# facebookresearch/video-long-term-feature-banks

Hardware: AMD Instinct MI355X
Metric: clips/sec fwd+bwd R50-I3D-NL+LFB-NL, 32x224^2 synthetic (higher is better)
Workload: dtype mix; 1 GPU; ava_r50_lfb_nl fwd+bwd+allreduce+sgd, 8 clips/GPU (global batch 8), RoIs/clip ~ U{1..5} (33 on rank 0), 32x224x224 clips; parallelism=dp1

## Files before the change

video-long-term-feature-banks_amd/csrc/vlfb_gemm.hip:

```cpp
#include "vlfb_conv_plan.h"
#include "vlfb_gemm_nt.h"

namespace vlfb {
namespace {

__device__ __forceinline__ uint32_t word_of(const uint4& v, int i) {
  return i == 0 ? v.x : i == 1 ? v.y : i == 2 ? v.z : v.w;
}
__device__ __forceinline__ void transpose_block(const uint4 (&in)[8], uint4 (&out)[8], bf16_t) {
#pragma unroll
  for (int c = 0; c < 8; ++c) {
    uint32_t o[4];
#pragma unroll
    for (int q = 0; q < 4; ++q) {
      const uint32_t w0 = word_of(in[2 * q], c >> 1), w1 = word_of(in[2 * q + 1], c >> 1);
      o[q] = (c & 1) ? ((w0 >> 16) | (w1 & 0xffff0000u)) : ((w0 & 0xffffu) | (w1 << 16));
    }
    out[c] = make_uint4(o[0], o[1], o[2], o[3]);
  }
}
__device__ __forceinline__ void transpose_block(const uint4 (&in)[8], uint4 (&out)[8], f16_t) {
  transpose_block(in, out, bf16_t());
}
__device__ __forceinline__ void transpose_block(const uint4 (&in)[4], uint4 (&out)[4], float) {
// ... 561 lines not shown
  float* slab = p.ws + (long long)split * ((long long)p.Ncols * p.ldo);
#pragma unroll
  for (int j = 0; j < kStemCT; ++j) {
    const int ct = ct0 + j;
    if (ct >= ncts) continue;
#pragma unroll
    for (int i = 0; i < 4; ++i) {
      const int co = i * 16 + l15;
      *reinterpret_cast<float4*>(slab + (long long)co * p.ldo + ct * 16 + g * 4) =
          make_float4(acc[j][i][0], acc[j][i][1], acc[j][i][2], acc[j][i][3]);
    }
  }
}

template <typename OutT, int G, int CL>
__global__ __launch_bounds__(CL * G) void wgrad_reduce_kernel(const float* ws, char* O, const float* rowscale,
                                                              long long n, int ldo, int splits, float alpha,
                                                              int accumulate, const float* __restrict__ ws_b = nullptr,
                                                              float* __restrict__ dbias = nullptr, int nb = 0, int wblocks = 0) {
  if (ws_b != nullptr && (int)blockIdx.x >= wblocks) {
    const int i = ((int)blockIdx.x - wblocks) * (CL * G) + (int)threadIdx.x;
    if (i < nb) {
      float s = 0.f;
      for (int k = 0; k < splits; ++k) s += ws_b[(long long)k * nb + i];
      dbias[i] = s * alpha * (rowscale ? rowscale[i] : 1.f);
    }
    return;
  }
  __shared__ float4 part[G > 1 ? (G - 1) * CL : 1];
  const int lane = threadIdx.x % CL, g = threadIdx.x / CL;
  const long long i = ((long long)blockIdx.x * CL + lane) * 4;
  float4 s = {0.f, 0.f, 0.f, 0.f};
  if (i < n) {
    const float* src = ws + i;
    int k = g;
    for (; k + 3 * G < splits; k += 4 * G) {
      float4 t0 = *reinterpret_cast<const float4*>(src + (long long)k * n);
      float4 t1 = *reinterpret_cast<const float4*>(src + (long long)(k + G) * n);
      float4 t2 = *reinterpret_cast<const float4*>(src + (long long)(k + 2 * G) * n);
      float4 t3 = *reinterpret_cast<const float4*>(src + (long long)(k + 3 * G) * n);
      s.x += (t0.x + t1.x) + (t2.x + t3.x); s.y += (t0.y + t1.y) + (t2.y + t3.y);
      s.z += (t0.z + t1.z) + (t2.z + t3.z); s.w += (t0.w + t1.w) + (t2.w + t3.w);
    }
    for (; k < splits; k += G) {
      float4 t = *reinterpret_cast<const float4*>(src + (long long)k * n);
      s.x += t.x; s.y += t.y; s.z += t.z; s.w += t.w;
    }
  }
  if (G > 1) {
    if (g > 0) part[(g - 1) * CL + lane] = s;
    __syncthreads();
    if (g == 0) {
#pragma unroll
      for (int j = 0; j < G - 1; ++j) {
        float4 t = part[j * CL + lane];
        s.x += t.x; s.y += t.y; s.z += t.z; s.w += t.w;
      }
    }
  }
  if (g == 0 && i < n) {
    float rs = alpha * (rowscale ? rowscale[i / ldo] : 1.f);
    float v[4] = {s.x * rs, s.y * rs, s.z * rs, s.w * rs};
    if (accumulate) {
#pragma unroll
      for (int r = 0; r < 4; ++r) v[r] += ld_elem<OutT>(O, i + r);
    }
    store4<OutT>(O, i, v, 4, true);
  }
}

__global__ void wgrad_bias_reduce_kernel(const float* __restrict__ ws_b, float* __restrict__ out,
                                         const float* __restrict__ rowscale, int n, int splits, float alpha) {
  const int i = blockIdx.x * blockDim.x + threadIdx.x;
  if (i >= n) return;
  float s = 0.f;
  for (int k = 0; k < splits; ++k) s += ws_b[(long long)k * n + i];
  out[i] = s * alpha * (rowscale ? rowscale[i] : 1.f);
}

template <auto Kernel>
int launch_k(const Plan& pl, hipStream_t s, const char* what) {
  return launch_lds<Kernel, 80 * 1024>(pl.grid, dim3(pl.threads), pl.lds, s, what, pl.gp);
}
template <typename T, typename OutT, int BM, int BN, bool IDENT, bool DGRAD, bool PACKW, int RB, bool PRE, int NW>
int launch_nt_shape(const Plan& pl, hipStream_t s, const char* what) {
  if constexpr (!IDENT && !PACKW) {
    if constexpr (DGRAD && sizeof(T) == 2) {
      if (pl.w2i) return launch_k<gemm_nt_kernel<T, OutT, BM, BN, IDENT, DGRAD, PACKW, RB, PRE, NW, 2, true, false, true>>(pl, s, what);
    }
    if (pl.ut) return launch_k<gemm_nt_kernel<T, OutT, BM, BN, IDENT, DGRAD, PACKW, RB, PRE, NW, 2, true>>(pl, s, what);
  }
  return launch_k<gemm_nt_kernel<T, OutT, BM, BN, IDENT, DGRAD, PACKW, RB, PRE, NW, 2, false>>(pl, s, what);
}

template <typename T, typename OutT, bool IDENT, bool DGRAD, bool PACKW>
int launch_nt(const Plan& pl, hipStream_t s, const char* what) {
  constexpr bool BF = sizeof(T) == 2;
  constexpr bool CAN_PRE = BF && sizeof(OutT) == 2 && !PACKW;
  constexpr int NW = BF ? 8 : 4;
  if (pl.bn == 64) {
    if (CAN_PRE && pl.pre) return launch_nt_shape<T, OutT, 128, 64, IDENT, DGRAD, PACKW, 128, CAN_PRE, NW>(pl, s, what);
    return launch_nt_shape<T, OutT, 128, 64, IDENT, DGRAD, PACKW, 128, false, NW>(pl, s, what);
  }
  if (CAN_PRE && pl.pre) return launch_nt_shape<T, OutT, 128, 128, IDENT, DGRAD, PACKW, 128, CAN_PRE, NW>(pl, s, what);
  return launch_nt_shape<T, OutT, 128, 128, IDENT, DGRAD, PACKW, 128, false, NW>(pl, s, what);
}
template <typename T, typename OutT, bool IDENT, bool PACKW>
int launch_tn(const Plan& pl, hipStream_t s, const char* what) {
  if (pl.bm == 128 && pl.bn == 128) return launch_k<gemm_tn_kernel<T, OutT, 128, 128, IDENT, PACKW>>(pl, s, what);
  if (pl.bm == 64 && pl.bn == 256) return launch_k<gemm_tn_kernel<T, OutT, 64, 256, IDENT, PACKW>>(pl, s, what);
  if (pl.bm == 64 && pl.bn == 128) return launch_k<gemm_tn_kernel<T, OutT, 64, 128, IDENT, PACKW>>(pl, s, what);
  if (pl.bm == 128 && pl.bn == 64) return launch_k<gemm_tn_kernel<T, OutT, 128, 64, IDENT, PACKW>>(pl, s, what);
  return launch_k<gemm_tn_kernel<T, OutT, 64, 64, IDENT, PACKW>>(pl, s, what);
}

template <typename T, typename OutT, bool IDENT, bool PACKW, bool SP>
int launch_tn_tr_as(const Plan& pl, hipStream_t s, const char* what) {
  if (pl.bm == 128 && pl.bn == 128) return launch_k<gemm_tn_tr_kernel<T, OutT, 128, 128, IDENT, PACKW, 8, SP>>(pl, s, what);
  if (pl.bm == 64 && pl.bn == 128) return launch_k<gemm_tn_tr_kernel<T, OutT, 64, 128, IDENT, PACKW, 4, SP>>(pl, s, what);
  if (pl.bm == 128 && pl.bn == 64) return launch_k<gemm_tn_tr_kernel<T, OutT, 128, 64, IDENT, PACKW, 4, SP>>(pl, s, what);
  return launch_k<gemm_tn_tr_kernel<T, OutT, 64, 64, IDENT, PACKW, 4, SP>>(pl, s, what);
}
template <typename T, typename OutT, bool SP = false>
int launch_tn_tr(const Plan& pl, hipStream_t s, const char* what) {
  return pl.ident ? launch_tn_tr_as<T, OutT, true, false, SP>(pl, s, what)
         : pl.packw ? launch_tn_tr_as<T, OutT, false, true, SP>(pl, s, what)
                    : launch_tn_tr_as<T, OutT, false, false, SP>(pl, s, what);
}

template <typename T>
int launch_stem_wgrad(const Plan& pl, hipStream_t s) {
  return launch_lds<stem_wgrad_kernel<T>, 160 * 1024>(pl.grid, dim3(512), pl.lds, s, "conv wgrad (stem) kernel", pl.gp);
}

template <typename T, typename OutT>
int launch_tiled(const vlfb_conv_desc* d, const Plan& pl, hipStream_t s) {
  if constexpr (sizeof(T) == 2) {
    if (pl.family == Family::tn_tr) return launch_tn_tr<T, OutT>(pl, s, "conv wgrad (tr) kernel");
  }
  const char* what = "conv kernel";
  if (d->mode == VLFB_CONV_WGRAD) {
    if (pl.ident) return launch_tn<T, OutT, true, false>(pl, s, what);
    if (pl.packw) return launch_tn<T, OutT, false, true>(pl, s, what);
    return launch_tn<T, OutT, false, false>(pl, s, what);
  }
  if (d->mode == VLFB_CONV_DGRAD) {
    if (pl.ident) return launch_nt<T, OutT, true, false, false>(pl, s, what);
    return launch_nt<T, OutT, false, true, false>(pl, s, what);
  }
  if (pl.ident) return launch_nt<T, OutT, true, false, false>(pl, s, what);
  if (pl.packw) return launch_nt<T, OutT, false, false, true>(pl, s, what);
  return launch_nt<T, OutT, false, false, false>(pl, s, what);
}

int launch_plan(const vlfb_conv_desc* d, const Plan& pl, hipStream_t s) {
  const GP& g = pl.gp;
  const bool out_f32 = d->out_dtype == VLFB_F32;
  switch (pl.family) {
    case Family::tn:
    case Family::tn_tr:
    case Family::nt:
      if (d->dtype == VLFB_F32) return launch_tiled<float, float>(d, pl, s);
      if (d->dtype == VLFB_F16) return out_f32 ? launch_tiled<f16_t, float>(d, pl, s) : launch_tiled<f16_t, f16_t>(d, pl, s);
      return out_f32 ? launch_tiled<bf16_t, float>(d, pl, s) : launch_tiled<bf16_t, bf16_t>(d, pl, s);
    case Family::tn8: return launch_tn8(g, pl.grid, d->dtype, out_f32, s);
    case Family::stem_wgrad: VLFB_WITH_T16(d->dtype, return launch_stem_wgrad<T16>(pl, s));
    case Family::wgrad_rows: return launch_wgrad_rows(g, pl.splits, pl.lds, d->dtype, s);
    case Family::wgrad_rows_fat: return launch_wgrad_rows_fat(g, pl.splits, d->dtype, s);
    case Family::tn_split: return launch_tn_split(g, pl.bm, pl.bn, pl.ident, pl.packw, pl.grid, pl.lds, s);
    case Family::tn_tr_planes: return launch_tn_tr<bf16_t, float, true>(pl, s, "conv wgrad (planes) kernel");
    case Family::nt8:
      return launch_nt8(g, pl.bm, pl.bn, pl.nt8_mode, d->dtype, out_f32, (unsigned)(d->batch > 0 ? d->batch : 1), s);
    case Family::nt_stream: return launch_nts(g, pl.nts_mode, d->dtype, s);
    case Family::conv_rows64: return launch_conv_rows64(g, d->mode, d->dtype, s);
    case Family::stem_fprop: return launch_stem_fprop(g, d->dtype, s);
    case Family::nt_skinny: return launch_skinny_nt(g, d->dtype, out_f32, s);
    case Family::nt_skinny_split: return launch_skinny_nt_split(g, s);
    case Family::nt_split: return launch_nt_split(g, pl.sp, pl.bn, pl.sp_kind, pl.ut != 0, pl.grid, pl.lds, s);
    case Family::nt_planes: return launch_nt_planes(g, pl.sp, pl.bn, pl.sp_kind, pl.grid, pl.lds, s);
    case Family::nt_pair: return launch_nt_pair(g, pl.bn, pl.ident, pl.pre != 0, out_f32, pl.grid, pl.lds, s);
    case Family::nt8_pair: return launch_nt8_pair(g, pl.bm, pl.bn, pl.nt8_mode, out_f32, s);
    case Family::stem_fprop_pair: return launch_stem_fprop_pair(g, s);
  }
  return set_error(VLFB_ERR_ARG, "conv: plan without a kernel family");
}

}
// ... 39 lines not shown
      const int64_t* v = static_cast<const int64_t*>(arg);
      const int64_t n = vlfb_class_ap_voc_workspace_bytes_impl(v[0], v[1]);
      if (n < 0) set_error(VLFB_ERR_ARG, "query_workspace: class_ap_voc needs 1 <= n <= %d and cols >= 1", VLFB_CLASS_AP_MAX_N);
      return n;
    }
    default: set_error(VLFB_ERR_ARG, "query_workspace: unknown op %d", op); return -1;
  }
}

extern "C" int vlfb_conv_run(const vlfb_conv_desc* d, const void* A, const void* B, const void* P,
                             void* O, const float* bias, const float* rowscale, const void* R,
                             const void* Mask, void* workspace, int64_t workspace_bytes,
                             vlfb_stream_t stream) {
  return vlfb_conv_run_planes(d, A, B, P, O, bias, rowscale, R, Mask, workspace, workspace_bytes, nullptr, stream);
}

static int conv_run_impl(const vlfb_conv_desc* d, const void* A, const void* B, const void* P,
                         void* O, const float* bias, const float* rowscale, const void* R,
                         const void* Mask, void* workspace, int64_t workspace_bytes, void* O_planes, float* dbias,
                         vlfb_stream_t stream, const void* R_lo = nullptr, void* O_lo = nullptr);

extern "C" int vlfb_conv_run_args(const vlfb_conv_desc* d, const vlfb_conv_args* a, vlfb_stream_t stream) {
  VLFB_REQUIRE(d && a, "conv_run_args: descriptor and arguments are required");
  VLFB_REQUIRE(!d->wgrad_bias == !a->dbias, "conv_run_args: dbias goes with desc.wgrad_bias");
  return conv_run_impl(d, a->A, a->B, a->P, a->O, a->bias, a->rowscale, a->R, a->Mask, a->workspace, a->workspace_bytes,
                       a->O_planes, a->dbias, stream, a->R_lo, a->O_lo);
}

extern "C" int vlfb_conv_run_planes(const vlfb_conv_desc* d, const void* A, const void* B, const void* P,
                                    void* O, const float* bias, const float* rowscale, const void* R,
                                    const void* Mask, void* workspace, int64_t workspace_bytes, void* O_planes,
                                    vlfb_stream_t stream) {
  VLFB_REQUIRE(!d->wgrad_bias, "conv: a descriptor with wgrad_bias runs through vlfb_conv_run_wgrad_bias");
  return conv_run_impl(d, A, B, P, O, bias, rowscale, R, Mask, workspace, workspace_bytes, O_planes, nullptr, stream);
}

extern "C" int vlfb_conv_run_wgrad_bias(const vlfb_conv_desc* d, const void* A, const void* P, void* O, float* dbias,
                                        const float* rowscale, void* workspace, int64_t workspace_bytes,
                                        vlfb_stream_t stream) {
  VLFB_REQUIRE(d->mode == VLFB_CONV_WGRAD && d->wgrad_bias && dbias, "conv_run_wgrad_bias: a WGRAD descriptor with wgrad_bias = 1 and dbias");
  return conv_run_impl(d, A, nullptr, P, O, nullptr, rowscale, nullptr, nullptr, workspace, workspace_bytes, nullptr, dbias, stream);
}

static int conv_run_impl(const vlfb_conv_desc* d, const void* A, const void* B, const void* P,
                         void* O, const float* bias, const float* rowscale, const void* R,
                         const void* Mask, void* workspace, int64_t workspace_bytes, void* O_planes, float* dbias,
                         vlfb_stream_t stream, const void* R_lo, void* O_lo) {
  Plan pl;
  int rc = cached_plan(d, &pl);
  if (rc != VLFB_OK) return rc;
  const bool h2 = d->math == VLFB_MATH_F16X3;
  const bool sp_pair = pl.sp && d->out_dtype == VLFB_F16;
  VLFB_REQUIRE(!sp_pair || (O_lo && (!R || R_lo)), "conv: a two-plane fp16 output needs O_lo (and R_lo with R)");
  VLFB_REQUIRE(!h2 || d->out_dtype == VLFB_F32 || O_lo, "conv: F16X3 math with a 16-bit output writes two planes (O, O_lo)");
  VLFB_REQUIRE(!h2 || !Mask, "conv: F16X3 launches take no mask");
  const bool copy16 = O_lo && !R_lo && !pl.sp && !h2 && is16(d->dtype) && d->out_dtype == VLFB_F32 && d->mode != VLFB_CONV_WGRAD;
  if ((R_lo || O_lo) && !sp_pair && !(h2 && d->out_dtype == VLFB_F32 && !R_lo)) {
    VLFB_REQUIRE(d->mode != VLFB_CONV_WGRAD && is16(d->dtype) && (d->out_dtype == d->dtype || copy16) && !pl.sp,
                 "conv: R_lo / O_lo belong to 16-bit FPROP / DGRAD launches with 16-bit outputs (O_lo alone: also with an fp32 output)");
    VLFB_REQUIRE(!R_lo || R, "conv: R_lo without R");
    VLFB_REQUIRE(pl.gp.vec_epi, "conv: R_lo / O_lo need 16-byte aligned output rows");
  }
  VLFB_REQUIRE(A && O, "conv: A and O are required");
  if (d->mode == VLFB_CONV_WGRAD) VLFB_REQUIRE(P != nullptr, "conv: WGRAD needs P");
  else VLFB_REQUIRE(B != nullptr, "conv: FPROP/DGRAD need B");
  VLFB_REQUIRE(d->bias_mode == VLFB_BIAS_NONE || bias != nullptr, "conv: bias_mode set but bias is NULL");
  if (pl.ws_elems > 0 && (workspace == nullptr || workspace_bytes < pl.ws_elems * 4))
    return set_error(VLFB_ERR_WORKSPACE, "conv: split WGRAD needs %lld workspace bytes, got %lld",
                     (long long)pl.ws_elems * 4, (long long)workspace_bytes);
  VLFB_REQUIRE((d->o_planes > 0) == (O_planes != nullptr), "conv: O_planes goes with desc.o_planes");
  rc = resolve_for_operands(d, &pl, R != nullptr, Mask != nullptr, R_lo != nullptr, O_lo != nullptr);
  if (rc != VLFB_OK) return rc;
  GP& g = pl.gp;
  g.A = (const char*)A; g.B = (const char*)B; g.P = (const char*)P; g.O = (char*)O;
  g.bias = bias; g.rowscale = rowscale; g.R = (const char*)R; g.Mask = (const char*)Mask;
  g.ws = (float*)workspace;
  g.OP = (char*)O_planes;
  g.dbias = pl.bias_fused ? dbias : nullptr;
  g.R2 = (const char*)R_lo; g.O2 = (char*)O_lo;
  g.pair_io = sp_pair ? 1 : 0;
  static const int nt_epi = env_int("VLFB_NT_EPI", 1);
  const bool wide_epi = h2 || pl.sp || pl.w2i || d->dt == 0 || d->out_dtype == VLFB_F32 || R_lo || O_lo;
  g.nt_epi = nt_epi >= 2 || (nt_epi == 1 && wide_epi);
  hipStream_t s = (hipStream_t)stream;
  rc = launch_plan(d, pl, s);
  if (rc != VLFB_OK) return rc;
  if (dbias && !pl.bias_fused) {
    VLFB_REQUIRE(!d->a_planes, "conv: wgrad_bias with pre-split operands is not supported (pass the fp32 operands)");
    const int slabs = colsum_slabs(d->dtype, g.M, d->Cn);
    float* part = g.ws + (pl.splits > 1 ? (long long)pl.splits * ((long long)d->Cn * g.ldo) : 0);
    rc = colsum_partials(P, d->dtype, g.M, d->Cn, g.ldp, part, s);
    if (rc != VLFB_OK) return rc;
    hipLaunchKernelGGL(wgrad_bias_reduce_kernel, dim3((unsigned)((d->Cn + 63) / 64)), dim3(64), 0, s, part, dbias, rowscale,
                       d->Cn, slabs, d->alpha);
  }
  const float* bias_rows = (dbias && pl.bias_fused && pl.splits > 1) ? g.ws + (long long)pl.splits * ((long long)d->Cn * g.ldo) : nullptr;
  if (pl.splits > 1) {
    const long long n = (long long)d->Cn * g.K;
    VLFB_REQUIRE(n % 4 == 0, "conv: split WGRAD output size must be a multiple of 4");
    const int G = pl.splits >= 32 ? 16 : pl.splits >= 8 ? 4 : 1;
#define VLFB_REDUCE(OT, GG, CC)                                                                                         \
  do {                                                                                                                  \
    const unsigned wblocks = (unsigned)((n / 4 + CC - 1) / CC);                                                         \
    const unsigned bblocks = bias_rows ? (unsigned)((d->Cn + CC * GG - 1) / (CC * GG)) : 0u;                            \
    hipLaunchKernelGGL((wgrad_reduce_kernel<OT, GG, CC>), dim3(wblocks + bblocks), dim3(CC * GG), 0, s, g.ws, g.O,     \
                       rowscale, n, g.ldo, pl.splits, d->alpha, d->accumulate, bias_rows, bias_rows ? dbias : nullptr,  \
                       (int)d->Cn, (int)wblocks);                                                                       \
  } while (0)
    with_elem(d->out_dtype, [&](auto t) {
      using OT = decltype(t);
      if (G == 16) VLFB_REDUCE(OT, 16, 16); else if (G == 4) VLFB_REDUCE(OT, 4, 64); else VLFB_REDUCE(OT, 1, 64);
    });
#undef VLFB_REDUCE
    return check_launch("wgrad reduce");
  }
  return VLFB_OK;
}
```

video-long-term-feature-banks_amd/csrc/vlfb_gemm_common.h:

```cpp
#pragma once
#include "vlfb_common.h"
#include <string.h>
#include <stdlib.h>

namespace vlfb {

struct GP {
  const char* A;
  const char* B;
  const char* P;
  char* O;
  const float* bias;
  const float* rowscale;
  const char* R;
  const char* Mask;
  float* ws;
  int M, Ncols, K;
  int Tr, Hr, Wr, Ts, Hs, Ws, Cs;
  int kt, kh, kw;
  float inv_khw, inv_kw, inv_kh;
  int st, sh, sw, pt, ph, pw, dt, dh, dw;
  int lst, lsh, lsw;
  int cpt_shift;
  int lda, ldb, ldo, ldr, ldp;
  long long a_bs, b_bs, o_bs, r_bs, p_bs;
  float alpha;
  int relu, bias_mode, accumulate;
  int tiles_m, tiles_n;
  int splits, kper;
  unsigned a_bytes, b_bytes;
  int vec_epi;
  int epi;
  int s2;
  int s2_mq;
  int s2_tpc;
  long long b_ps;
  long long a_ps, p_ps, o_ps;
  char* OP;
  int op_n;
  float* dbias;
  const char* R2;
  char* O2;
  int pair_io;
  int nt_epi;
};

int launch_nt8(const GP& gp, int bm, int bn, int mode, int dtype, bool out_f32, unsigned batch, hipStream_t s);
int launch_tn8(const GP& gp, dim3 grid, int dtype, bool out_f32, hipStream_t s);

int nts_chunk(int mode, long long K);
int launch_nts(const GP& gp, int mode, int dtype, hipStream_t s);

int wgrad_rows_ct(long long K);
int launch_wgrad_rows(const GP& gp, int splits, size_t lds, int dtype, hipStream_t s);
int launch_wgrad_rows_fat(const GP& gp, int splits, int dtype, hipStream_t s);

bool skinny_nt_ok(const GP& gp, int dtype, long long batch, bool ident);
int launch_skinny_nt(const GP& gp, int dtype, bool out_f32, hipStream_t s);
bool skinny_nt_split_ok(const GP& gp, long long batch, bool ident);
int launch_skinny_nt_split(const GP& gp, hipStream_t s);

bool stem_fprop_ok(const GP& gp, int pack_w, int dtype, int out_dtype, long long batch);
int launch_stem_fprop(const GP& gp, int dtype, hipStream_t s);
bool stem_fprop_pair_ok(const GP& gp, int pack_w, long long batch);
int launch_stem_fprop_pair(const GP& gp, hipStream_t s);

bool conv_rows64_ok(const GP& gp, int mode, int dtype, int out_dtype, long long batch);
int launch_conv_rows64(const GP& gp, int mode, int dtype, hipStream_t s);

int launch_nt_split(const GP& gp, int npl, int bn, int kind, bool ut, dim3 grid, size_t lds, hipStream_t s);
int launch_tn_split(const GP& gp, int bp, int bq, bool ident, bool packw, dim3 grid, size_t lds, hipStream_t s);
int launch_nt_planes(const GP& gp, int npl, int bn, int kind, dim3 grid, size_t lds, hipStream_t s);
int launch_nt_pair(const GP& gp, int bn, bool ident, bool pre, bool out_f32, dim3 grid, size_t lds, hipStream_t s);
int launch_nt8_pair(const GP& gp, int bm, int bn, int mode, bool out_f32, hipStream_t s);

namespace {

typedef __attribute__((ext_vector_type(8))) __bf16 bf16x8_v;
typedef __attribute__((ext_vector_type(8))) _Float16 f16x8_v;
typedef __attribute__((ext_vector_type(4))) float f32x4_v;

constexpr int kThreads = 256;
constexpr int kRowBytes = 128;
constexpr int kStemCT = 9;


struct RowC { int n, t, h, w; };

__device__ __forceinline__ RowC decode_row(const GP& p, int m) {
  RowC r;
  int hw = p.Hr * p.Wr;
  int thw = p.Tr * hw;
  r.n = m / thw;
  int rem = m - r.n * thw;
  r.t = rem / hw;
  rem -= r.t * hw;
  r.h = rem / p.Wr;
  r.w = rem - r.h * p.Wr;
  return r;
}
__device__ __forceinline__ void advance_row(const GP& p, RowC& r) {
  if (++r.w == p.Wr) {
    r.w = 0;
    if (++r.h == p.Hr) {
      r.h = 0;
      if (++r.t == p.Tr) { r.t = 0; ++r.n; }
    }
  }
}

struct TapC { int a, b, c, ci; bool ok; };

template <typename T, bool PACKW>
__device__ __forceinline__ TapC decode_tap(const GP& p, int kc) {
  constexpr int EPC = Elem<T>::EPC;
  TapC t;
  t.ok = kc * EPC < p.K;
  int tap = kc >> p.cpt_shift;
  int within = kc & ((1 << p.cpt_shift) - 1);
  if (PACKW) {
    t.a = (int)(((float)tap + 0.5f) * p.inv_kh);
    t.b = tap - t.a * p.kh;
    t.c = within * (EPC / 4);
    t.ci = 0;
  } else {
    t.a = (int)(((float)tap + 0.5f) * p.inv_khw);
    int rem = tap - t.a * p.kh * p.kw;
// ... 235 lines not shown
```

video-long-term-feature-banks_amd/csrc/vlfb_gemm_nt.h:

```cpp
#pragma once
#include "vlfb_gemm_common.h"

namespace vlfb {
namespace {

template <typename T, typename OutT, int BM, int BN, bool IDENT, bool DGRAD, bool PACKW, int RB, bool PRE, int NW,
          int ST = 2, bool UT = false, bool PAIR = false, bool W2I = false>
__global__ __launch_bounds__(64 * NW) void gemm_nt_kernel(const GP p) {
  static_assert(!W2I || (sizeof(T) == 2 && RB == 128 && ST == 2 && UT && DGRAD && !PAIR), "W2I: 16-bit unit-stride DGRAD on the tap cursor");
  static_assert(!PAIR || (sizeof(T) == 2 && RB == 128 && ST == 2 && (IDENT || UT) && !PACKW && !DGRAD), "PAIR: fp16 planes, plain rows or UT FPROP");
  static_assert(!UT || (!IDENT && !PACKW), "UT is for gathered, unpacked operands");
  constexpr int NTHR = 64 * NW;
  constexpr int NWN = NW / 2;
  constexpr int EPC = Elem<T>::EPC;
  constexpr int CPRW = RB / 16;
  constexpr int RPPS = NTHR / CPRW;
  constexpr int A_IT = BM / RPPS, B_IT = BN / RPPS;
  constexpr int WM = BM / 2, WN = BN / NWN;
  constexpr int FM = WM / 16, FN = WN / 16;
  constexpr int BUF = (BM + BN) * RB;
  constexpr int KSTEPS = sizeof(T) == 4 ? 1 : RB / 64;
  extern __shared__ __attribute__((aligned(16))) char smem[];

  const int tid = threadIdx.x, lane = tid & 63, wave = tid >> 6;
  const int wm = wave / NWN, wn = wave % NWN;
  const int l15 = lane & 15, g = lane >> 4;

  const int nwg = p.tiles_m * p.tiles_n;
  const int bid = xcd_remap(blockIdx.x, nwg);
  const int tile_m = bid / p.tiles_n, tile_n = bid - tile_m * p.tiles_n;
  int m0 = tile_m * BM;
  const int n0 = tile_n * BN;
  const int z = blockIdx.z;
  constexpr bool S2C = DGRAD && !UT && !IDENT && !PACKW;
  bool s2 = false;
  int s2_ph = 0, s2_pw = 0;
  if constexpr (S2C) {
    s2 = p.s2 != 0;
    if (s2) {
      const int cls = tile_m / p.s2_tpc;
      m0 = (tile_m - cls * p.s2_tpc) * BM;
      s2_ph = cls >> 1; s2_pw = cls & 1;
    }
  }
  const int mrows = s2 ? p.s2_mq : p.M;
  auto row_coords = [&](int m) {
    if constexpr (S2C) {
      if (s2) {
        const int w2n = p.Wr >> 1, h2n = p.Hr >> 1;
        RowC r;
        const int w2 = m % w2n; int q = m / w2n;
        const int h2 = q % h2n; q /= h2n;
        r.t = q % p.Tr; r.n = q / p.Tr;
        r.h = 2 * h2 + s2_ph; r.w = 2 * w2 + s2_pw;
        return r;
      }
    }
    return decode_row(p, m);
  };
  auto row_pos = [&](int m) -> long long {
    if constexpr (S2C) {
      if (s2) {
        const RowC r = row_coords(m);
        return (long long)((r.n * p.Tr + r.t) * p.Hr + r.h) * p.Wr + r.w;
      }
    }
    return m;
  };

  const char* Ab = p.A + (long long)z * p.a_bs * (long long)sizeof(T);
  const char* Bb = p.B + (long long)z * p.b_bs * (long long)sizeof(T);

  const int cc = tid % CPRW;
  const int r0 = tid / CPRW;
  const int ccg = cc ^ swz_key<RB>(r0);
  const unsigned a_cb = PAIR ? (unsigned)(ccg & 3) * 16u + (unsigned)(ccg >> 2) * (unsigned)p.a_ps * 2u : (unsigned)(ccg * EPC) * (unsigned)sizeof(T);
  const unsigned b_cb = PAIR ? (unsigned)(ccg & 3) * 16u + (unsigned)(ccg >> 2) * (unsigned)p.b_ps * 2u : (unsigned)(ccg * EPC) * (unsigned)sizeof(T);
  const int KTB = PAIR ? RB / 2 : RB;
  const int wave_u = __builtin_amdgcn_readfirstlane(wave);

  RowC arow[A_IT];
  bool aok[A_IT];
  int upix[UT ? A_IT : 1];
#pragma unroll
  for (int i = 0; i < A_IT; ++i) {
    int m = m0 + r0 + RPPS * i;
    aok[i] = m < mrows;
    if (!IDENT) arow[i] = row_coords(aok[i] ? m : 0);
    if (UT) {
      RowC& r = arow[i];
// ... 47 lines not shown
    int kt = kt_seq;
    if constexpr (S2C) {
      if (s2) kt = s2_next_kt();
    }
    const int kc = PAIR ? kt * (CPRW / 2) + (ccg & 3) : kt * CPRW + ccg;
    TapC tap;
    if (IDENT || UT) { tap.ok = kc * EPC < p.K; tap.a = tap.b = tap.c = tap.ci = 0; }
    else tap = decode_tap<T, PACKW>(p, kc);
    const bool kok = W2I || kc * EPC < p.K;
    {
      char* xa = smem + (W2I ? (kt_seq >> 1) & 1 : buf) * BUF + wave_u * 1024;
      char* wb = smem + buf * BUF + BM * RB + wave_u * 1024;
      const unsigned kbyte = (unsigned)kt * KTB;
      if (UT) {
        const int sgn = DGRAD ? -1 : 1;
        const int da = sgn * u_a * p.dt, db = sgn * u_b * p.dh, dc = sgn * u_c * p.dw;
        const unsigned dbyte = (unsigned)(((da * p.Hs + db) * p.Ws + dc) * p.lda + u_ci) * (unsigned)sizeof(T);
        if (!W2I || !(kt_seq & 1)) {
#pragma unroll
          for (int i = 0; i < A_IT; ++i) {
            const bool ok = aok[i] && (unsigned)(arow[i].t + da) < (unsigned)p.Ts &&
                            (unsigned)(arow[i].h + db) < (unsigned)p.Hs && (unsigned)(arow[i].w + dc) < (unsigned)p.Ws;
            bufglds16(rsA, ok ? aoff[i] + dbyte : kOOB, 0, xa + i * (RPPS * RB));
          }
          u_ci += (PAIR ? RB / 2 : RB) / (int)sizeof(T);
          if (u_ci >= p.Cs) {
            u_ci = 0;
            if (++u_c == p.kw) { u_c = 0; if (++u_b == p.kh) { u_b = 0; ++u_a; } }
          }
        }
      } else if (IDENT) {
#pragma unroll
        for (int i = 0; i < A_IT; ++i) bufglds16(rsA, kok ? aoff[i] : kOOB, kbyte, xa + i * (RPPS * RB));
      } else {
#pragma unroll
        for (int i = 0; i < A_IT; ++i) {
          unsigned off;
          if (PACKW) {
            const int ts = arow[i].t * p.st - p.pt + tap.a * p.dt;
            const int hs = arow[i].h * p.sh - p.ph + tap.b * p.dh;
            const bool ok = aok[i] && tap.ok && (unsigned)ts < (unsigned)p.Ts && (unsigned)hs < (unsigned)p.Hs;
            const int w0 = arow[i].w * p.sw - p.pw + tap.c;
            const int pix = ((arow[i].n * p.Ts + ts) * p.Hs + hs) * p.Ws + w0;
            off = ok ? (unsigned)pix * 4u * (unsigned)sizeof(T) : kOOB;
          } else {
            bool ok;
            const long long e = src_offset<DGRAD>(p, arow[i], tap, ok);
            off = (ok && aok[i] && tap.ok) ? (unsigned)e * (unsigned)sizeof(T) : kOOB;
          }
          bufglds16(rsA, off, 0, xa + i * (RPPS * RB));
        }
      }
#pragma unroll
      for (int i = 0; i < B_IT; ++i) bufglds16(rsB, kok ? boff[i] : kOOB, kbyte, wb + i * (RPPS * RB));
    }
  };
  constexpr int LPT = A_IT + B_IT;
  auto ring_wait = [&](int newer) {
    if (newer >= 3 && ST >= 5) asm volatile("s_waitcnt vmcnt(%0)" ::"n"(3 * LPT) : "memory");
    else if (newer == 2 && ST >= 4) asm volatile("s_waitcnt vmcnt(%0)" ::"n"(2 * LPT) : "memory");
    else if (newer == 1 && ST >= 3) asm volatile("s_waitcnt vmcnt(%0)" ::"n"(1 * LPT) : "memory");
    else asm volatile("s_waitcnt vmcnt(0)" ::: "memory");
  };

  f32x4_v acc[FN][FM];
#pragma unroll
  for (int a = 0; a < FN; ++a)
#pragma unroll
    for (int b = 0; b < FM; ++b) acc[a][b] = f32x4_v{0.f, 0.f, 0.f, 0.f};

  char* Ob = p.O + (long long)z * p.o_bs * (long long)sizeof(OutT);
  const char* Rb = p.R ? p.R + (long long)z * p.r_bs * (long long)sizeof(T) : nullptr;
  const char* Mb = p.Mask ? p.Mask + (long long)z * p.r_bs * (long long)sizeof(T) : nullptr;
  const char* R2b = p.R2 ? p.R2 + (long long)z * p.r_bs * (long long)sizeof(T) : nullptr;
  char* O2b = p.O2 ? p.O2 + (long long)z * p.o_bs * ((PAIR || sizeof(T) == 2) ? 2ll : (long long)sizeof(OutT)) : nullptr;
  constexpr int EPT = 16 / (int)sizeof(OutT);
  constexpr int TPR = BN / EPT;
  constexpr int RPP = NTHR / TPR;
  constexpr int NPASS = BM / RPP;
  const int tc = tid % TPR, tr = tid / TPR;
  const int ncol = n0 + tc * EPT;
  constexpr bool PREM = PRE && !PAIR;
  constexpr bool PRE2 = PRE && PAIR;
  const bool nt = p.nt_epi != 0;
  uint4 rpre[PRE ? NPASS : 1], mpre[PREM ? NPASS : 1], r2pre[PRE2 ? NPASS : 1];
  if (PRE) {
#pragma unroll
    for (int gp = 0; gp < NPASS; ++gp) {
      const int m = m0 + gp * RPP + tr;
      const bool ok = m < mrows && ncol < p.Ncols;
      const long long off = (row_pos(ok ? m : 0) * p.ldr + ncol) * (long long)sizeof(T);
      rpre[gp] = ld16_epi(nt, src_or_zero(Rb ? Rb : Ab, off, ok && Rb != nullptr));
      if constexpr (PRE2) r2pre[gp] = ld16_epi(nt, src_or_zero(R2b ? R2b : Ab, off, ok && R2b != nullptr));
      if constexpr (PREM) mpre[gp] = ld16_epi(nt, src_or_zero(Mb ? Mb : Ab, off, ok && Mb != nullptr));
    }
  }
  (void)R2b; (void)O2b;

  static_assert(ST >= 2 && ST <= 5 && 3 * LPT < 64, "ring depth / vmcnt immediate");
#pragma unroll
  for (int s0 = 0; s0 < ST - 1; ++s0)
    if (s0 < ktiles) load_tile(s0, s0);

  int cur = 0, nxt = ST - 1;
  if constexpr (W2I) {
    constexpr bool HOLD = !PRE;
    for (int kt = 0; kt < ktiles; kt += 2) {
      typename Mma<T>::Frag xf[KSTEPS][FM];
      asm volatile("s_waitcnt vmcnt(0)" ::: "memory");
      asm volatile("s_barrier" ::: "memory");
      load_tile(kt + 1, 1);
      {
        const char* xa = smem + ((kt >> 1) & 1) * BUF;
        const char* wb = smem + BM * RB;
        if constexpr (HOLD) {
#pragma unroll
          for (int ks = 0; ks < KSTEPS; ++ks)
#pragma unroll
            for (int i = 0; i < FM; ++i) xf[ks][i] = Mma<T>::template load<RB>(xa, wm * WM + i * 16 + l15, ks, g);
        }
#pragma unroll
        for (int ks = 0; ks < KSTEPS; ++ks) {
          typename Mma<T>::Frag wf[FN];
          if constexpr (!HOLD) {
#pragma unroll
            for (int i = 0; i < FM; ++i) xf[ks][i] = Mma<T>::template load<RB>(xa, wm * WM + i * 16 + l15, ks, g);
          }
#pragma unroll
          for (int j = 0; j < FN; ++j) wf[j] = Mma<T>::template load<RB>(wb, wn * WN + j * 16 + l15, ks, g);
#pragma unroll
          for (int j = 0; j < FN; ++j)
#pragma unroll
            for (int i = 0; i < FM; ++i) acc[j][i] = Mma<T>::mma(wf[j], xf[ks][i], acc[j][i]);
        }
      }
      asm volatile("s_waitcnt vmcnt(0)" ::: "memory");
      asm volatile("s_barrier" ::: "memory");
      if (kt + 2 < ktiles) load_tile(kt + 2, 0);
      {
        const char* xa = smem + ((kt >> 1) & 1) * BUF;
        const char* wb = smem + BUF + BM * RB;
#pragma unroll
        for (int ks = 0; ks < KSTEPS; ++ks) {
          typename Mma<T>::Frag wf[FN];
          if constexpr (!HOLD) {
#pragma unroll
            for (int i = 0; i < FM; ++i) xf[ks][i] = Mma<T>::template load<RB>(xa, wm * WM + i * 16 + l15, ks, g);
          }
#pragma unroll
          for (int j = 0; j < FN; ++j) wf[j] = Mma<T>::template load<RB>(wb, wn * WN + j * 16 + l15, ks, g);
#pragma unroll
          for (int j = 0; j < FN; ++j)
#pragma unroll
            for (int i = 0; i < FM; ++i) acc[j][i] = Mma<T>::mma(wf[j], xf[ks][i], acc[j][i]);
        }
      }
    }
  } else
  for (int kt = 0; kt < ktiles; ++kt) {
    const int ahead = ktiles - 1 - kt;
    ring_wait(ahead < ST - 2 ? ahead : ST - 2);
    asm volatile("s_barrier" ::: "memory");
    const bool more = kt + ST - 1 < ktiles;
    if (more) load_tile(kt + ST - 1, nxt);
    const char* xa = smem + cur * BUF;
    const char* wb = xa + BM * RB;
    if constexpr (PAIR) {
      typename Mma<T>::Frag xh[FM], xl[FM], wh[FN], wl[FN];
#pragma unroll
      for (int i = 0; i < FM; ++i) {
        xh[i] = Mma<T>::template load<RB>(xa, wm * WM + i * 16 + l15, 0, g);
        xl[i] = Mma<T>::template load<RB>(xa, wm * WM + i * 16 + l15, 1, g);
      }
#pragma unroll
      for (int j = 0; j < FN; ++j) {
        wh[j] = Mma<T>::template load<RB>(wb, wn * WN + j * 16 + l15, 0, g);
        wl[j] = Mma<T>::template load<RB>(wb, wn * WN + j * 16 + l15, 1, g);
      }
#pragma unroll
      for (int j = 0; j < FN; ++j)
#pragma unroll
        for (int i = 0; i < FM; ++i) acc[j][i] = Mma<T>::mma(wl[j], xh[i], acc[j][i]);
#pragma unroll
      for (int j = 0; j < FN; ++j)
#pragma unroll
        for (int i = 0; i < FM; ++i) acc[j][i] = Mma<T>::mma(wh[j], xl[i], acc[j][i]);
#pragma unroll
      for (int j = 0; j < FN; ++j)
#pragma unroll
        for (int i = 0; i < FM; ++i) acc[j][i] = Mma<T>::mma(wh[j], xh[i], acc[j][i]);
    } else {
#pragma unroll
    for (int ks = 0; ks < KSTEPS; ++ks) {
      typename Mma<T>::Frag xf[FM], wf[FN];
#pragma unroll
      for (int i = 0; i < FM; ++i) xf[i] = Mma<T>::template load<RB>(xa, wm * WM + i * 16 + l15, ks, g);
#pragma unroll
      for (int j = 0; j < FN; ++j) wf[j] = Mma<T>::template load<RB>(wb, wn * WN + j * 16 + l15, ks, g);
#pragma unroll
      for (int j = 0; j < FN; ++j)
#pragma unroll
        for (int i = 0; i < FM; ++i) acc[j][i] = Mma<T>::mma(wf[j], xf[i], acc[j][i]);
    }
    }
    cur = cur + 1 == ST ? 0 : cur + 1;
    nxt = nxt + 1 == ST ? 0 : nxt + 1;
  }
  __syncthreads();

  if (p.vec_epi) {
    constexpr int CPR = BN / 4;
    const int epi = p.epi;
    auto stage = [&](int h) {
      if (epi == 1 || wm == h) {
#pragma unroll
        for (int i = 0; i < FM; ++i) {
          const int row = (epi == 1 ? wm * WM : 0) + i * 16 + l15;
#pragma unroll
          for (int j = 0; j < FN; ++j) {
            const int c = (wn * WN + j * 16 + g * 4) >> 2;
            *reinterpret_cast<float4*>(smem + ((row * CPR + (c ^ (row & 7))) << 4)) =
                make_float4(acc[j][i][0] * p.alpha, acc[j][i][1] * p.alpha, acc[j][i][2] * p.alpha,
                            acc[j][i][3] * p.alpha);
          }
        }
      }
    };
    stage(0);
    __syncthreads();
#pragma unroll
    for (int gp = 0; gp < NPASS; ++gp) {
      if (gp == NPASS / 2 && epi == 2) {
        __syncthreads();
        stage(1);
        __syncthreads();
      }
      const int trow = gp * RPP + tr;
      const int row = (epi == 2 && gp >= NPASS / 2) ? trow - BM / 2 : trow;
      const int m = m0 + trow;
      if (m < mrows && ncol < p.Ncols) {
        const long long mpos = row_pos(m);
        float v[EPT];
#pragma unroll
        for (int q = 0; q < EPT / 4; ++q) {
          const int c = tc * (EPT / 4) + q;
          const float4 t = *reinterpret_cast<const float4*>(smem + ((row * CPR + (c ^ (row & 7))) << 4));
          v[4 * q] = t.x; v[4 * q + 1] = t.y; v[4 * q + 2] = t.z; v[4 * q + 3] = t.w;
// ... 95 lines not shown
```

video-long-term-feature-banks_amd/csrc/vlfb_gemm_pair.hip:

```cpp
#include "vlfb_gemm_nt.h"
#include "vlfb_gemm_nt8.h"

namespace vlfb {
namespace {

template <auto Kernel>
int launch_pair_k(dim3 grid, int threads, size_t lds, const GP& gp, hipStream_t s) {
  return launch_lds<Kernel, 80 * 1024>(grid, dim3(threads), lds, s, "conv kernel (fp16 planes)", gp);
}

template <typename OutT, int BN, bool PRE>
int launch_pair_shape(const GP& gp, bool ident, dim3 grid, size_t lds, hipStream_t s) {
  constexpr int NW = 8;
  if (ident) return launch_pair_k<gemm_nt_kernel<f16_t, OutT, 128, BN, true, false, false, 128, PRE, NW, 2, false, true>>(grid, 64 * NW, lds, gp, s);
  return launch_pair_k<gemm_nt_kernel<f16_t, OutT, 128, BN, false, false, false, 128, PRE, NW, 2, true, true>>(grid, 64 * NW, lds, gp, s);
}

template <auto Kernel>
int launch_pair8_k(const GP& gp, dim3 grid, size_t lds, hipStream_t s) {
  return launch_lds<Kernel, 160 * 1024>(grid, dim3(512), lds, s, "conv kernel (fp16 planes, 256-row pipelined)", gp);
}
template <typename OutT, int BN, int RV>
int launch_pair8_bn(const GP& gp, int mode, dim3 grid, hipStream_t s) {
  constexpr size_t lds = (BN == 256 ? 2 : 3) * (size_t)(2 + BN / 128) * 16384;
  if (mode == 0) return launch_pair8_k<gemm_nt8_kernel<f16_t, OutT, BN, 0, false, RV, true>>(gp, grid, lds, s);
  return launch_pair8_k<gemm_nt8_kernel<f16_t, OutT, BN, 1, false, RV, true>>(gp, grid, lds, s);
}
template <typename OutT>
int launch_pair8_t(const GP& gp, int mode, int bm, int bn, dim3 grid, hipStream_t s) {
  if (bn == 256) return bm == 196 ? launch_pair8_bn<OutT, 256, 98>(gp, mode, grid, s) : launch_pair8_bn<OutT, 256, 128>(gp, mode, grid, s);
  return bm == 196 ? launch_pair8_bn<OutT, 128, 98>(gp, mode, grid, s) : launch_pair8_bn<OutT, 128, 128>(gp, mode, grid, s);
}

}

int launch_nt8_pair(const GP& gp, int bm, int bn, int mode, bool out_f32, hipStream_t s) {
  const dim3 grid((unsigned)(gp.tiles_m * gp.tiles_n), 1, 1);
  return out_f32 ? launch_pair8_t<float>(gp, mode, bm, bn, grid, s) : launch_pair8_t<f16_t>(gp, mode, bm, bn, grid, s);
}

int launch_nt_pair(const GP& gp, int bn, bool ident, bool pre, bool out_f32, dim3 grid, size_t lds, hipStream_t s) {
  if (out_f32) {
    if (bn == 64) return launch_pair_shape<float, 64, false>(gp, ident, grid, lds, s);
    return launch_pair_shape<float, 128, false>(gp, ident, grid, lds, s);
  }
  if (pre) {
    if (bn == 64) return launch_pair_shape<f16_t, 64, true>(gp, ident, grid, lds, s);
    return launch_pair_shape<f16_t, 128, true>(gp, ident, grid, lds, s);
  }
  if (bn == 64) return launch_pair_shape<f16_t, 64, false>(gp, ident, grid, lds, s);
  return launch_pair_shape<f16_t, 128, false>(gp, ident, grid, lds, s);
}

}
```

Baseline: 266.9 clips/s.

## Stream epilogue residual/mask prefetch behind K-loop tile loads in NT GEMM

Instead of issuing every residual, mask and second-residual prefetch load before the main loop, the PRE variant now issues one pass of them after each tile load and waits with a vmcnt budget that leaves those slices in flight. This spreads epilogue prefetch traffic across the K loop so it does not delay the first tiles, and it is on by default through VLFB_PRE_STREAM. It also adds a template flag so these prefetches use nontemporal loads when the nontemporal epilogue is selected, and it marks the main loops nounroll. The cost is more template instantiations and tighter vmcnt reasoning, which could go wrong if the wait counts do not match the number of loads actually issued.

```diff
diff --git a/video-long-term-feature-banks_amd/csrc/vlfb_gemm.hip b/video-long-term-feature-banks_amd/csrc/vlfb_gemm.hip
--- a/video-long-term-feature-banks_amd/csrc/vlfb_gemm.hip
+++ b/video-long-term-feature-banks_amd/csrc/vlfb_gemm.hip
@@ -667,15 +667,20 @@
 int launch_k(const Plan& pl, hipStream_t s, const char* what) {
   return launch_lds<Kernel, 80 * 1024>(pl.grid, dim3(pl.threads), pl.lds, s, what, pl.gp);
 }
-template <typename T, typename OutT, int BM, int BN, bool IDENT, bool DGRAD, bool PACKW, int RB, bool PRE, int NW>
+template <typename T, typename OutT, int BM, int BN, bool IDENT, bool DGRAD, bool PACKW, int RB, bool PRE, int NW, bool NTP = false>
 int launch_nt_shape(const Plan& pl, hipStream_t s, const char* what) {
   if constexpr (!IDENT && !PACKW) {
     if constexpr (DGRAD && sizeof(T) == 2) {
-      if (pl.w2i) return launch_k<gemm_nt_kernel<T, OutT, BM, BN, IDENT, DGRAD, PACKW, RB, PRE, NW, 2, true, false, true>>(pl, s, what);
-    }
-    if (pl.ut) return launch_k<gemm_nt_kernel<T, OutT, BM, BN, IDENT, DGRAD, PACKW, RB, PRE, NW, 2, true>>(pl, s, what);
-  }
-  return launch_k<gemm_nt_kernel<T, OutT, BM, BN, IDENT, DGRAD, PACKW, RB, PRE, NW, 2, false>>(pl, s, what);
+      if (pl.w2i) return launch_k<gemm_nt_kernel<T, OutT, BM, BN, IDENT, DGRAD, PACKW, RB, PRE, NW, 2, true, false, true, NTP>>(pl, s, what);
+    }
+    if (pl.ut) return launch_k<gemm_nt_kernel<T, OutT, BM, BN, IDENT, DGRAD, PACKW, RB, PRE, NW, 2, true, false, false, NTP>>(pl, s, what);
+  }
+  return launch_k<gemm_nt_kernel<T, OutT, BM, BN, IDENT, DGRAD, PACKW, RB, PRE, NW, 2, false, false, false, NTP>>(pl, s, what);
+}
+template <typename T, typename OutT, int BN, bool IDENT, bool DGRAD, bool PACKW, int NW>
+int launch_nt_pre(const Plan& pl, hipStream_t s, const char* what) {
+  if (pl.gp.nt_epi) return launch_nt_shape<T, OutT, 128, BN, IDENT, DGRAD, PACKW, 128, true, NW, true>(pl, s, what);
+  return launch_nt_shape<T, OutT, 128, BN, IDENT, DGRAD, PACKW, 128, true, NW, false>(pl, s, what);
 }
 
 template <typename T, typename OutT, bool IDENT, bool DGRAD, bool PACKW>
@@ -684,10 +689,10 @@
   constexpr bool CAN_PRE = BF && sizeof(OutT) == 2 && !PACKW;
   constexpr int NW = BF ? 8 : 4;
   if (pl.bn == 64) {
-    if (CAN_PRE && pl.pre) return launch_nt_shape<T, OutT, 128, 64, IDENT, DGRAD, PACKW, 128, CAN_PRE, NW>(pl, s, what);
+    if constexpr (CAN_PRE) { if (pl.pre) return launch_nt_pre<T, OutT, 64, IDENT, DGRAD, PACKW, NW>(pl, s, what); }
     return launch_nt_shape<T, OutT, 128, 64, IDENT, DGRAD, PACKW, 128, false, NW>(pl, s, what);
   }
-  if (CAN_PRE && pl.pre) return launch_nt_shape<T, OutT, 128, 128, IDENT, DGRAD, PACKW, 128, CAN_PRE, NW>(pl, s, what);
+  if constexpr (CAN_PRE) { if (pl.pre) return launch_nt_pre<T, OutT, 128, IDENT, DGRAD, PACKW, NW>(pl, s, what); }
   return launch_nt_shape<T, OutT, 128, 128, IDENT, DGRAD, PACKW, 128, false, NW>(pl, s, what);
 }
 template <typename T, typename OutT, bool IDENT, bool PACKW>
@@ -893,6 +898,8 @@
   static const int nt_epi = env_int("VLFB_NT_EPI", 1);
   const bool wide_epi = h2 || pl.sp || pl.w2i || d->dt == 0 || d->out_dtype == VLFB_F32 || R_lo || O_lo;
   g.nt_epi = nt_epi >= 2 || (nt_epi == 1 && wide_epi);
+  static const int pre_stream = env_int("VLFB_PRE_STREAM", 1);
+  g.pre_stream = pre_stream != 0;
   hipStream_t s = (hipStream_t)stream;
   rc = launch_plan(d, pl, s);
   if (rc != VLFB_OK) return rc;
diff --git a/video-long-term-feature-banks_amd/csrc/vlfb_gemm_common.h b/video-long-term-feature-banks_amd/csrc/vlfb_gemm_common.h
--- a/video-long-term-feature-banks_amd/csrc/vlfb_gemm_common.h
+++ b/video-long-term-feature-banks_amd/csrc/vlfb_gemm_common.h
@@ -43,6 +43,7 @@
   char* O2;
   int pair_io;
   int nt_epi;
+  int pre_stream;
 };
 
 int launch_nt8(const GP& gp, int bm, int bn, int mode, int dtype, bool out_f32, unsigned batch, hipStream_t s);
diff --git a/video-long-term-feature-banks_amd/csrc/vlfb_gemm_nt.h b/video-long-term-feature-banks_amd/csrc/vlfb_gemm_nt.h
--- a/video-long-term-feature-banks_amd/csrc/vlfb_gemm_nt.h
+++ b/video-long-term-feature-banks_amd/csrc/vlfb_gemm_nt.h
@@ -5,7 +5,7 @@
 namespace {
 
 template <typename T, typename OutT, int BM, int BN, bool IDENT, bool DGRAD, bool PACKW, int RB, bool PRE, int NW,
-          int ST = 2, bool UT = false, bool PAIR = false, bool W2I = false>
+          int ST = 2, bool UT = false, bool PAIR = false, bool W2I = false, bool NTP = false>
 __global__ __launch_bounds__(64 * NW) void gemm_nt_kernel(const GP p) {
   static_assert(!W2I || (sizeof(T) == 2 && RB == 128 && ST == 2 && UT && DGRAD && !PAIR), "W2I: 16-bit unit-stride DGRAD on the tap cursor");
   static_assert(!PAIR || (sizeof(T) == 2 && RB == 128 && ST == 2 && (IDENT || UT) && !PACKW && !DGRAD), "PAIR: fp16 planes, plain rows or UT FPROP");
@@ -219,18 +219,60 @@
   const int ncol = n0 + tc * EPT;
   constexpr bool PREM = PRE && !PAIR;
   constexpr bool PRE2 = PRE && PAIR;
+  constexpr int SL = 1 + (PREM ? 1 : 0) + (PRE2 ? 1 : 0);
+  static_assert(!PRE || ST == 2, "PRE slices: one tile in flight");
+  static_assert(LPT + SL < 64, "tile + slice in flight / vmcnt immediate");
   const bool nt = p.nt_epi != 0;
+  const bool pre_stream = PRE && p.pre_stream != 0;
   uint4 rpre[PRE ? NPASS : 1], mpre[PREM ? NPASS : 1], r2pre[PRE2 ? NPASS : 1];
-  if (PRE) {
+  static_assert(PRE || !NTP, "NTP belongs to the PRE rows");
+  int pre_on = 1;
+  if constexpr (PRE) {
+    asm volatile("" : "+s"(pre_on));
 #pragma unroll
     for (int gp = 0; gp < NPASS; ++gp) {
-      const int m = m0 + gp * RPP + tr;
-      const bool ok = m < mrows && ncol < p.Ncols;
-      const long long off = (row_pos(ok ? m : 0) * p.ldr + ncol) * (long long)sizeof(T);
-      rpre[gp] = ld16_epi(nt, src_or_zero(Rb ? Rb : Ab, off, ok && Rb != nullptr));
-      if constexpr (PRE2) r2pre[gp] = ld16_epi(nt, src_or_zero(R2b ? R2b : Ab, off, ok && R2b != nullptr));
-      if constexpr (PREM) mpre[gp] = ld16_epi(nt, src_or_zero(Mb ? Mb : Ab, off, ok && Mb != nullptr));
-    }
+      rpre[gp] = make_uint4(0u, 0u, 0u, 0u);
+      if constexpr (PRE2) r2pre[gp] = make_uint4(0u, 0u, 0u, 0u);
+      if constexpr (PREM) mpre[gp] = make_uint4(0u, 0u, 0u, 0u);
+    }
+  }
+  auto pre_load = [&](uint4& dst, const char* src) {
+    asm volatile("" : "+v"(src));
+    const auto* gsrc = (const __attribute__((address_space(1))) u32x4_vec*)(size_t)src;
+    if (pre_on) {
+      u32x4_vec t;
+      if constexpr (NTP) t = __builtin_nontemporal_load(gsrc);
+      else t = *gsrc;
+      dst = make_uint4(t.x, t.y, t.z, t.w);
+    }
+  };
+  auto pre_request = [&](int lo, int hi) {
+    int tid_s = tid;
+    asm volatile("" : "+v"(tid_s));
+    const int tr_s = tid_s / TPR, ncol_s = n0 + (tid_s % TPR) * EPT;
+#pragma unroll
+    for (int gp = 0; gp < NPASS; ++gp) {
+      if (gp >= lo && gp < hi) {
+        const int m = m0 + gp * RPP + tr_s;
+        const bool ok = m < mrows && ncol_s < p.Ncols;
+        const long long off = (row_pos(ok ? m : 0) * p.ldr + ncol_s) * (long long)sizeof(T);
+        pre_load(rpre[PRE ? gp : 0], src_or_zero(Rb ? Rb : Ab, off, ok && Rb != nullptr));
+        if constexpr (PRE2) pre_load(r2pre[gp], src_or_zero(R2b ? R2b : Ab, off, ok && R2b != nullptr));
+        if constexpr (PREM) pre_load(mpre[gp], src_or_zero(Mb ? Mb : Ab, off, ok && Mb != nullptr));
+      }
+    }
+  };
+  auto pre_behind = [&](int s) {
+    if constexpr (PRE) {
+      if (pre_stream && s < NPASS) pre_request(s, s + 1 >= ktiles ? NPASS : s + 1);
+    }
+  };
+  auto pre_wait = [&](int kt) {
+    if (PRE && pre_stream && kt < NPASS) asm volatile("s_waitcnt vmcnt(%0)" ::"n"(SL) : "memory");
+    else asm volatile("s_waitcnt vmcnt(0)" ::: "memory");
+  };
+  if constexpr (PRE) {
+    if (!pre_stream) pre_request(0, NPASS);
   }
   (void)R2b; (void)O2b;
 
@@ -238,15 +280,18 @@
 #pragma unroll
   for (int s0 = 0; s0 < ST - 1; ++s0)
     if (s0 < ktiles) load_tile(s0, s0);
+  pre_behind(0);
 
   int cur = 0, nxt = ST - 1;
   if constexpr (W2I) {
     constexpr bool HOLD = !PRE;
+#pragma nounroll
     for (int kt = 0; kt < ktiles; kt += 2) {
       typename Mma<T>::Frag xf[KSTEPS][FM];
-      asm volatile("s_waitcnt vmcnt(0)" ::: "memory");
+      pre_wait(kt);
       asm volatile("s_barrier" ::: "memory");
       load_tile(kt + 1, 1);
+      pre_behind(kt + 1);
       {
         const char* xa = smem + ((kt >> 1) & 1) * BUF;
         const char* wb = smem + BM * RB;
@@ -271,9 +316,9 @@
             for (int i = 0; i < FM; ++i) acc[j][i] = Mma<T>::mma(wf[j], xf[ks][i], acc[j][i]);
         }
       }
-      asm volatile("s_waitcnt vmcnt(0)" ::: "memory");
+      pre_wait(kt + 1);
       asm volatile("s_barrier" ::: "memory");
-      if (kt + 2 < ktiles) load_tile(kt + 2, 0);
+      if (kt + 2 < ktiles) { load_tile(kt + 2, 0); pre_behind(kt + 2); }
       {
         const char* xa = smem + ((kt >> 1) & 1) * BUF;
         const char* wb = smem + BUF + BM * RB;
@@ -294,12 +339,14 @@
       }
     }
   } else
+#pragma nounroll
   for (int kt = 0; kt < ktiles; ++kt) {
     const int ahead = ktiles - 1 - kt;
-    ring_wait(ahead < ST - 2 ? ahead : ST - 2);
+    if constexpr (PRE) pre_wait(kt);
+    else ring_wait(ahead < ST - 2 ? ahead : ST - 2);
     asm volatile("s_barrier" ::: "memory");
     const bool more = kt + ST - 1 < ktiles;
-    if (more) load_tile(kt + ST - 1, nxt);
+    if (more) { load_tile(kt + ST - 1, nxt); pre_behind(kt + ST - 1); }
     const char* xa = smem + cur * BUF;
     const char* wb = xa + BM * RB;
     if constexpr (PAIR) {
diff --git a/video-long-term-feature-banks_amd/csrc/vlfb_gemm_pair.hip b/video-long-term-feature-banks_amd/csrc/vlfb_gemm_pair.hip
--- a/video-long-term-feature-banks_amd/csrc/vlfb_gemm_pair.hip
+++ b/video-long-term-feature-banks_amd/csrc/vlfb_gemm_pair.hip
@@ -9,11 +9,11 @@
   return launch_lds<Kernel, 80 * 1024>(grid, dim3(threads), lds, s, "conv kernel (fp16 planes)", gp);
 }
 
-template <typename OutT, int BN, bool PRE>
+template <typename OutT, int BN, bool PRE, bool NTP = false>
 int launch_pair_shape(const GP& gp, bool ident, dim3 grid, size_t lds, hipStream_t s) {
   constexpr int NW = 8;
-  if (ident) return launch_pair_k<gemm_nt_kernel<f16_t, OutT, 128, BN, true, false, false, 128, PRE, NW, 2, false, true>>(grid, 64 * NW, lds, gp, s);
-  return launch_pair_k<gemm_nt_kernel<f16_t, OutT, 128, BN, false, false, false, 128, PRE, NW, 2, true, true>>(grid, 64 * NW, lds, gp, s);
+  if (ident) return launch_pair_k<gemm_nt_kernel<f16_t, OutT, 128, BN, true, false, false, 128, PRE, NW, 2, false, true, false, NTP>>(grid, 64 * NW, lds, gp, s);
+  return launch_pair_k<gemm_nt_kernel<f16_t, OutT, 128, BN, false, false, false, 128, PRE, NW, 2, true, true, false, NTP>>(grid, 64 * NW, lds, gp, s);
 }
 
 template <auto Kernel>
@@ -45,8 +45,8 @@
     return launch_pair_shape<float, 128, false>(gp, ident, grid, lds, s);
   }
   if (pre) {
-    if (bn == 64) return launch_pair_shape<f16_t, 64, true>(gp, ident, grid, lds, s);
-    return launch_pair_shape<f16_t, 128, true>(gp, ident, grid, lds, s);
+    if (bn == 64) return gp.nt_epi ? launch_pair_shape<f16_t, 64, true, true>(gp, ident, grid, lds, s) : launch_pair_shape<f16_t, 64, true, false>(gp, ident, grid, lds, s);
+    return gp.nt_epi ? launch_pair_shape<f16_t, 128, true, true>(gp, ident, grid, lds, s) : launch_pair_shape<f16_t, 128, true, false>(gp, ident, grid, lds, s);
   }
   if (bn == 64) return launch_pair_shape<f16_t, 64, false>(gp, ident, grid, lds, s);
   return launch_pair_shape<f16_t, 128, false>(gp, ident, grid, lds, s);
```

Result: no change. 266.7 clips/s (-0.1%).
